# kimweiskopf/fargocpt

Measured on AMD Instinct MI355X. Metric: cell-updates/s on Nr x Nphi polar grid, higher is better.
Workload: dtype f64

## Files before the change

### fargocpt_amd/binding.py

```python
from __future__ import annotations

import ctypes as C
from typing import Optional

import numpy as np

ABI_VERSION = 5
OVERLAP = 7
GEOM_PAD = 15
MAX_BODIES = 8
NBODY_STATE = 9

SPACING_ARITHMETIC, SPACING_LOGARITHMIC, SPACING_EXPONENTIAL = 0, 1, 2
EOS_ISOTHERMAL, EOS_IDEAL = 0, 1
ARTVISC_NONE, ARTVISC_TW, ARTVISC_SN = 0, 1, 2
OPACITY_LIN, OPACITY_BELL, OPACITY_CONST, OPACITY_SIMPLE = 0, 1, 2, 3
BETAREF_ZERO, BETAREF_REFERENCE, BETAREF_MODEL, BETAREF_FLOOR = 0, 1, 2, 3
LIMITER_VANLEER, LIMITER_MC = 0, 1
INTEGRATOR_EULER, INTEGRATOR_LEAPFROG = 0, 1
(BC_ZEROGRADIENT, BC_REFERENCE, BC_REFLECTING, BC_OUTFLOW, BC_KEPLERIAN, BC_ZEROSHEAR,
 BC_NONE) = range(7)
DAMP_NONE, DAMP_REFERENCE, DAMP_ZERO, DAMP_MEAN = range(4)
IC_PROFILE, IC_SPREADING_RING, IC_SHOCKTUBE = range(3)
(F_SIGMA, F_VRAD, F_VAZI, F_ENERGY, F_PRESSURE, F_SOUNDSPEED, F_SCALE_HEIGHT, F_VISCOSITY,
 F_TEMPERATURE, F_POTENTIAL, F_SIGMA0, F_VRAD0, F_VAZI0, F_ENERGY0, F_QPLUS, F_QMINUS,
 F_VISC_CFAC_PHI, F_VISC_CFAC_R, F_MASSFLOW, F_ACCEL_RADIAL, F_ACCEL_AZIMUTHAL) = range(21)
VECTOR_FIELDS = (F_VRAD, F_VRAD0, F_MASSFLOW, F_ACCEL_RADIAL, F_ACCEL_AZIMUTHAL)
COMM_ID_BYTES = 128

ERRORS = {-1: "FCPT_EINVAL", -2: "FCPT_ENOMEM", -3: "FCPT_EHIP", -4: "FCPT_ESPLIT", -5: "FCPT_ENODEV", -6: "FCPT_ESHEAR",
          -7: "FCPT_ECOMM"}

_i32, _u32, _u64, _f64 = C.c_int32, C.c_uint32, C.c_uint64, C.c_double


class Desc(C.Structure):
    _fields_ = [
        ("struct_size", _u32), ("abi_version", _u32),
        ("nr_global", _i32), ("nphi", _i32), ("rank", _i32), ("nranks", _i32),
        ("radial_spacing", _i32), ("_pad0", _i32),
        ("rmin", _f64), ("rmax", _f64), ("exponential_cell_size_factor", _f64),
        ("eos", _i32), ("_pad1", _i32),
        ("adiabatic_index", _f64), ("mu", _f64), ("aspect_ratio", _f64), ("flaring_index", _f64),
        ("minimum_temperature", _f64), ("maximum_temperature", _f64),
        ("sigma0", _f64), ("sigma_slope", _f64), ("sigma_floor", _f64),
        ("viscous_alpha", _f64), ("constant_viscosity", _f64), ("radial_viscosity_factor", _f64),
        ("stabilize_viscosity", _i32), ("artificial_viscosity", _i32),
        ("artificial_viscosity_factor", _f64),
        ("artificial_viscosity_dissipation", _i32), ("heating_viscous", _i32),
        ("heating_viscous_factor", _f64),
        ("fast_transport", _i32), ("flux_limiter", _i32),
        ("integrator", _i32), ("_pad2", _i32),
        ("cfl", _f64), ("cfl_max_var", _f64), ("first_dt", _f64),
        ("heating_cooling_cfl_limit", _f64), ("monitor_timestep", _f64),
# ... 461 lines not shown
```

### fargocpt_amd/csrc/fcpt_context.hip

```cpp
#include "fcpt_ctx.h"

using namespace fcpt;

namespace fcpt {

void drop_graph(fcpt_ctx *c)
{
    if (c->graph_exec)
        (void)hipGraphExecDestroy(c->graph_exec);
    if (c->graph)
        (void)hipGraphDestroy(c->graph);
    c->graph_exec = nullptr;
    c->graph = nullptr;
    c->graph_cycle = 0;
}

void join_side(fcpt_ctx *c)
{
    if (c->join_pending) {
        (void)hipStreamWaitEvent(c->stream, c->e_join, 0);
        c->join_pending = false;
    }
}

int read_clock(fcpt_ctx *c, DevClock *out)
{
    join_side(c);
    HIPCHK(hipMemcpyAsync(c->h_clk, c->P.clk, sizeof(DevClock), hipMemcpyDeviceToHost, c->stream));
    HIPCHK(hipStreamSynchronize(c->stream));
    *out = *c->h_clk;
    if (out->shear_error) {
        set_error("a step exceeded the FARGO shear limit (|Nshift[i]-Nshift[i-1]| > 1) with the option "
                  "transport_fallback = 0, i.e. without the two-kernel transport queued behind the fused one; "
                  "the state is invalid");
        return FCPT_ESHEAR;
    }
    return FCPT_OK;
}

}

namespace {

int *option_slot(Options &o, const char *name)
{
#define X(n)                     \
    if (!std::strcmp(name, #n)) \
        return &o.n;
    FCPT_OPTION_NAMES
#undef X
    return nullptr;
}

void options_from_environment(Options &o)
{
    o.transport_fused = o.transport_rows = o.source_rows = o.theta_rows = -1;
    o.transport_graded = 1;
    o.source_graded = -1;
// ... 406 lines not shown
                    R.ra1sq_k = ra1 * ra1;
                    R.ra0sq_k = ra0 * ra0;
                    R.inv_rmsum_k = 1.0 / (g.Rmed[k] + g.Rmed[k - 1]);
                    R.rmed_k = g.Rmed[k];
                    R.rmed_km1 = g.Rmed[k - 1];
                    R.idr_k = at(g.InvDiffRmed, k);
                }
            }
        }
        if (!rc) rc = dev_upload_raw(c, &P.src_tab, rows);
    }

    const size_t ns = (size_t)nr * nphi, nv = (size_t)(nr + 1) * nphi;
#define AL(field, n) \
    if (!rc)         \
        rc = dev_alloc(c, &P.field, (n));
    AL(sigma, ns) AL(vrad, nv) AL(vazi, ns) AL(energy, ns) AL(vrad_b, nv) AL(vazi_b, ns) AL(energy_b, ns)
    AL(pressure, ns) AL(soundspeed, ns) AL(scale_height, ns) AL(viscosity, ns) AL(temperature, ns)
    AL(potential, ns)
    AL(sigma0, ns) AL(vrad0, nv) AL(vazi0, ns) AL(energy0, ns)
    AL(qr, ns) AL(qphi, ns) AL(divv, ns) AL(trr, ns) AL(tpp, ns) AL(trp, nv) AL(qplus, ns) AL(qminus, ns)
    AL(rmpA, ns) AL(rmmA, ns) AL(lpA, ns) AL(lmA, ns) AL(sigA, ns) AL(eA, ns)
    AL(rmpB, ns) AL(rmmB, ns) AL(lpB, ns) AL(lmB, ns) AL(sigB, ns) AL(eB, ns)
    AL(vmean, (size_t)nr + 1) AL(vconst, (size_t)nr) AL(nshift, (size_t)nr) AL(clk, 1) AL(shift_jump, 8)
    AL(cfl_part, (size_t)(nr + 256) * (size_t)((nphi + 255) / 256 + 1))
    P.ring_pstride = nphi / 32 + 4;
    AL(ring_part, (size_t)nr * P.ring_pstride)
    P.stabilize = d->stabilize_viscosity;
    if (P.stabilize) {
        AL(cfac_phi, ns) AL(cfac_r, ns)
    }
    if (d->write_massflow) {
        AL(massflow, nv)
    }
    P.accel_force = d->body_force_from_potential ? 0 : 1;
    if (P.accel_force) {
        AL(accel_r, nv) AL(accel_az, nv)
    }
    if (!rc && d->eos == FCPT_EOS_IDEAL)
        rc = dev_alloc(c, &P.qdiff, ns);
#undef AL
    if (!rc && hipHostMalloc((void **)&c->h_clk, sizeof(DevClock)) != hipSuccess) {
        set_error("hipHostMalloc failed");
        rc = FCPT_ENOMEM;
    }
    if (rc) {
        fcpt_destroy(c);
// ... 215 lines not shown
    *slot = value;
    apply_options(c, false);
    HIPCHK(hipGetLastError());
    return FCPT_OK;
}

int fcpt_get_option(const fcpt_ctx *c, const char *name, int32_t *value)
{
    if (!c || !name || !value)
        return FCPT_EINVAL;
    if (!std::strcmp(name, "graph_replays")) {
        *value = (int32_t)(c->graph_replays > 0x7fffffffll ? 0x7fffffffll : c->graph_replays);
        return FCPT_OK;
    }
    if (!std::strcmp(name, "transport_fell_back")) {
        fcpt_ctx *m = const_cast<fcpt_ctx *>(c);
        int stamps[4] = {0, 0, 0, 0};
        join_side(m);
        HIPCHK(hipMemcpyAsync(stamps, c->P.shift_jump, sizeof(stamps), hipMemcpyDeviceToHost, c->stream));
        HIPCHK(hipStreamSynchronize(c->stream));
        *value = (stamps[2] != 0 && stamps[0] == stamps[2]) ? 1 : 0;
        return FCPT_OK;
    }
    if (!std::strcmp(name, "coop_active")) {
        *value = 0;
        return FCPT_OK;
    }
    if (!std::strcmp(name, "graph_cycle")) {
        *value = c->graph_exec ? c->graph_cycle : 0;
        return FCPT_OK;
    }
    const int *slot = option_slot(const_cast<Options &>(c->P.opt), name);
    if (!slot) {
        set_error("fcpt_get_option: unknown option '%s'", name);
        return FCPT_EINVAL;
    }
    *value = *slot;
    return FCPT_OK;
}

int fcpt_set_transport_chunks(fcpt_ctx *c, const int32_t *lengths, int32_t n)
{
    if (!c || n < 0 || (n > 0 && !lengths))
        return FCPT_EINVAL;
    if (c->stepped) {
        set_error("fcpt_set_transport_chunks between fcpt_step and fcpt_post");
// ... 120 lines not shown
        *dt_max = k.dt_max;
    if (reset) {
        k.dt_min = 1.0e300;
        k.dt_max = 0.0;
        *c->h_clk = k;
        HIPCHK(hipMemcpyAsync(c->P.clk, c->h_clk, sizeof(DevClock), hipMemcpyHostToDevice, c->stream));
        HIPCHK(hipStreamSynchronize(c->stream));
    }
    return FCPT_OK;
}

int fcpt_set_clock(fcpt_ctx *c, const fcpt_clock *in)
{
    if (!c || !in)
        return FCPT_EINVAL;
    DevClock k;
    if (int rc = read_clock(c, &k))
        return rc;
    k.time = in->time;
    k.last_dt = in->last_dt;
    k.n_hydro_iter = in->n_hydro_iter;
    k.n_monitor = in->n_monitor;
    k.n_snapshot = in->n_snapshot;
    HIPCHK(hipMemsetAsync(c->P.shift_jump, 0, 8 * sizeof(int), c->stream));
    *c->h_clk = k;
    HIPCHK(hipMemcpyAsync(c->P.clk, c->h_clk, sizeof(DevClock), hipMemcpyHostToDevice, c->stream));
    HIPCHK(hipStreamSynchronize(c->stream));
    return FCPT_OK;
}

static size_t grid_count(const fcpt_ctx *c, int32_t f)
{
    const bool vec = f == FCPT_F_VRAD || f == FCPT_F_VRAD0 || f == FCPT_F_MASSFLOW || f == FCPT_F_ACCEL_RADIAL ||
                     f == FCPT_F_ACCEL_AZIMUTHAL;
    return (size_t)(c->s.nr + (vec ? 1 : 0)) * c->d.nphi;
}

int fcpt_upload(fcpt_ctx *c, int32_t f, const double *host)
{
    if (!c || !host || f < 0 || f >= FCPT_F_COUNT || !c->grid[f]) {
        set_error("bad argument to fcpt_upload");
        return FCPT_EINVAL;
    }
    join_side(c);
    HIPCHK(hipMemcpyAsync(c->grid[f], host, grid_count(c, f) * sizeof(double), hipMemcpyHostToDevice, c->stream));
    HIPCHK(hipStreamSynchronize(c->stream));
    if (f == FCPT_F_SIGMA || f == FCPT_F_VRAD || f == FCPT_F_VAZI || f == FCPT_F_ENERGY) {
// ... 329 lines not shown
```

### fargocpt_amd/csrc/fcpt_ctx.h

```cpp
#ifndef FCPT_CTX_H
#define FCPT_CTX_H

#include <hip/hip_runtime.h>

#include <cmath>
#include <cstdio>
#include <cstdlib>
#include <cstring>
#include <new>
#include <string>
#include <vector>

#include "fcpt_comm.h"
#include "fcpt_kernels.h"

using namespace fcpt;

#define HIPCHK(call)                                                                        \
    do {                                                                                    \
        hipError_t e_ = (call);                                                             \
        if (e_ != hipSuccess) {                                                             \
            set_error("%s failed: %s (%s:%d)", #call, hipGetErrorString(e_), __FILE__, __LINE__); \
            return FCPT_EHIP;                                                               \
        }                                                                                   \
// ... 6 lines not shown
    std::vector<double> radii;
    Dev P;
    hipStream_t stream = nullptr;
    std::vector<void *> allocs;
    double *d_cs_ring = nullptr;
    double *grid[FCPT_F_COUNT] = {};
    DampRange damp[4][2];
    bool potential_valid = false;
    DevClock *h_clk = nullptr;
    Profiler prof;
    bool profiling = false;
    bool fused_source = true;
    int src_parts = 0;
    bool kick_energy_b = false;
    bool kick_bc_folded = false;
    bool ghosts_unknown = true;
    bool policy_dt_dev = false;
    double policy_dt_host = -1.0;
    bool march_source = true;
    bool stepped = false;
    bool bc_deferred = false;
    bool skip_q_store = false;
    bool want_gated_deferred = false, gated_pending = false;
    GatedTheta gated;
    bool fold_pending = false;
    bool cfl_interior = false;
    bool damp_any = false;
    bool qdiff_valid = false;
    std::vector<int> ring_ref_damped;
    int *sm_sched_dev = nullptr;
    size_t sm_sched_cap = 0;
    std::vector<int> sm_sched_host;
    int *tf_sched_dev = nullptr;
    size_t tf_sched_cap = 0;
    std::vector<int> tf_lengths;
    std::vector<int> tf_sched_host;
    bool damp_foldable = false;
    hipStream_t side = nullptr;
    hipEvent_t e_fork = nullptr, e_join = nullptr;
    bool join_pending = false;
    bool pressure_valid = false;
    double *dob_part = nullptr, *dob_host = nullptr;
    hipEvent_t e_dob = nullptr;
    int dob_pending = 0;
    bool has_mid = false;
    double mx[FCPT_MAX_BODIES], my[FCPT_MAX_BODIES], mm[FCPT_MAX_BODIES], mrsm[FCPT_MAX_BODIES];
// ... 75 lines not shown
```

### fargocpt_amd/csrc/fcpt_internal.h

```cpp
#ifndef FCPT_INTERNAL_H
#define FCPT_INTERNAL_H

#include "../../include/fargocpt_hip.h"

#include <cstddef>
#include <cstdint>
#include <vector>

#ifndef M_PI
#define M_PI 3.14159265358979323846
#endif

namespace fcpt {

void set_error(const char *fmt, ...);

struct HostGeometry {
    std::vector<double> Rmed, Rinf, Rsup, Surf, InvRmed, InvRinf, InvSurf, InvDiffRmed, InvDiffRsup,
        InvDiffRsupRb;
    double dphi = 0, invdphi = 0;
    double cf_growth = 0, cf_inv_log_growth = 0, cf_opt_const = 0;
};

int build_radii(const fcpt_desc &d, double *radii);
int split_domain(const fcpt_desc &d, fcpt_split &out);
void build_geometry(const fcpt_desc &d, const fcpt_split &s, const double *radii, HostGeometry &g);
int rmed_id(const fcpt_desc &d, const fcpt_split &s, const HostGeometry &g, double r);
int rinf_id(const fcpt_desc &d, const fcpt_split &s, const HostGeometry &g, double r);

struct DevClock {
    double time;
    double last_dt;
    double dt;
    double cfl_dt;
    unsigned long long cfl_bits;
    unsigned long long n_hydro_iter;
    unsigned int n_monitor;
    unsigned int n_snapshot;
    unsigned int shear_error;
    unsigned int last_dt_pending;
    double dt_min, dt_max;
};
#ifdef __HIPCC__
__device__ __forceinline__ void clock_advance(DevClock *clk, double dt)
{
    clk->time += dt;
    clk->n_hydro_iter += 1;
    if (clk->last_dt_pending) {
        clk->last_dt = dt;
        clk->last_dt_pending = 0;
    }
    clk->dt_min = dt < clk->dt_min ? dt : clk->dt_min;
    clk->dt_max = dt > clk->dt_max ? dt : clk->dt_max;
}
#endif

struct DampRange {
    int lo, hi;
    int type;
    double rlim, redge, tau;
};

struct CArr {
    const double *p;
// ... 166 lines not shown
```

### fargocpt_amd/csrc/fcpt_kernels.h

```cpp
#ifndef FCPT_KERNELS_H
#define FCPT_KERNELS_H

#include <vector>
#include <hip/hip_runtime.h>

#include "fcpt_internal.h"
#include "fcpt_schedule.h"

namespace fcpt {

enum KernelId {
    KID_POTENTIAL, KID_SOURCE_VR, KID_SOURCE_VA, KID_COMPRESSION, KID_TW_Q, KID_TW_VA, KID_TW_VR,
    KID_SN_Q, KID_SN_E, KID_SN_VR, KID_SN_VA, KID_TRANGE, KID_ADI_CS_H, KID_ISO_CS_H,
    KID_VISCOSITY, KID_PRESSURE, KID_TEMPERATURE, KID_STRESS_DIAG, KID_STRESS_RPHI, KID_VISC_VA,
    KID_VISC_VR, KID_QPLUS, KID_SUBSTEP3, KID_BOUNDARY, KID_DAMPING, KID_TRANSPORT_RADIAL,
    KID_RING_MEAN, KID_THETA1, KID_THETA2, KID_VELOCITIES, KID_CFL_INIT, KID_CFL_CELLS, KID_CLOCK,
    KID_SRC_FUSED, KID_AV_FUSED, KID_VISC_FUSED, KID_SOURCE_MARCH, KID_THETA_MARCH,
    KID_TRANSPORT_FUSED, KID_MASSFLOW, KID_CFL_RINGS, KID_THETA_GATED_BOUNDARY, KID_EXCHANGE_COPY,
    KID_DISK_ON_BODY, KID_VISC_FACTORS, KID_SOURCE_MARCH_ADI, KID_SOURCE_MARCH_ADI_WIDE,
    KID_ACCEL_ON_GAS, KID_SOURCE_MARCH_ADI_ACC, KID_TRANSPORT_RADIAL_MEANS, KID_CFL_RINGS_BC,
    KID_DISK_ON_BODIES, KID_COUNT
};
static_assert(KID_COUNT <= 64, "fcpt_profile_start selects kernels with a 64-bit mask");
extern const char *const kKernelNames[KID_COUNT];
// ... 41 lines not shown
TransportResult launch_transport(const Dev &P, const Dev &W, hipStream_t st, int part = TRANSPORT_ALL, GatedTheta *defer_gated = nullptr);
int device_cus();
void launch_shift_means(const Dev &P, hipStream_t st);
void launch_massflow(const Dev &P, hipStream_t st);
void launch_substep3_cooling_only(const Dev &P, hipStream_t st);
void launch_disk_on_body(const Dev &P, double x, double y, double r_object, double smoothing_fixed, double r_sm, double *out,
                         hipStream_t st);
struct DiskBodies {
    double x[FCPT_MAX_BODIES], y[FCPT_MAX_BODIES], r_object[FCPT_MAX_BODIES], smoothing_fixed[FCPT_MAX_BODIES], r_sm[FCPT_MAX_BODIES];
};
size_t disk_on_bodies_blocks(const Dev &P);
void launch_disk_on_bodies(const Dev &P, int n, const DiskBodies &B, double *part, double *out, hipStream_t st);
void launch_source_fused(const Dev &P, hipStream_t st);
int launch_source_march(const Dev &P, hipStream_t st, bool fold_bc, bool *bc_folded, bool fold_cfl = false);
void launch_cfl_final(const Dev &P, int apply_policy, hipStream_t st);
bool cfl_by_rings(const Dev &P);
void launch_viscous_fused(const Dev &P, hipStream_t st);
void launch_derived(const Dev &P, hipStream_t st);
void launch_pressure(const Dev &P, hipStream_t st);
void launch_temperature(const Dev &P, hipStream_t st);
void launch_cfl(const Dev &P, int apply_policy, hipStream_t st, bool interior_done = false);
bool launch_cfl_interior(const Dev &P, hipStream_t st);
bool cfl_bc_mergeable(const Dev &P);
void launch_cfl_bc(const Dev &P, int apply_policy, hipStream_t st);
void launch_clock_set_dt(DevClock *clk, double dt, hipStream_t st);
void launch_clock_scale_dt(DevClock *clk, int mode, double dt, double factor, hipStream_t st);
void launch_clock_export_cfl(DevClock *clk, double *out, hipStream_t st);
void launch_clock_policy_ptr(DevClock *clk, double cfl_max_var, const double *cfl_global, hipStream_t st);
void launch_clock_advance(DevClock *clk, hipStream_t st);
void launch_clock_policy(DevClock *clk, double cfl_max_var, int use_device_cfl, double cfl_global,
                         hipStream_t st);

}
#endif
```

### fargocpt_amd/csrc/fcpt_step.hip

```cpp
#include "fcpt_ctx.h"

using namespace fcpt;

namespace fcpt {

void apply_boundary_view(fcpt_ctx *c, const Dev &P, bool final, bool damping_done)
{
    if (final && c->d.damping && !damping_done) {
        for (int o = 0; o < 2; ++o)
            launch_damping(P, P.vrad, P.vrad0, P.Rinf.p, c->damp[0][o], 0, c->stream);
        for (int o = 0; o < 2; ++o)
            launch_damping(P, P.vazi, P.vazi0, P.Rmed.p, c->damp[1][o], 0, c->stream);
        for (int o = 0; o < 2; ++o)
            launch_damping(P, P.sigma, P.sigma0, P.Rmed.p, c->damp[2][o], 1, c->stream);
        if (P.adiabatic)
            for (int o = 0; o < 2; ++o)
                launch_damping(P, P.energy, P.energy0, P.Rmed.p, c->damp[3][o], 0, c->stream);
    }
    launch_boundary(P, c->stream);
}
void apply_boundary(fcpt_ctx *c, bool final) { apply_boundary_view(c, c->P, final); }

void ensure_pressure(fcpt_ctx *c)
{
// ... 164 lines not shown
        c->pressure_valid = false;
        if (P.adiabatic && !P.lazy_derived)
            ensure_pressure(c);
        c->P.kick_time_shift = 1;
        const bool home = enqueue_kick(c);
        c->P.kick_time_shift = 0;
        if (home) {
            const size_t ns = (size_t)P.nr * P.nphi * sizeof(double), nv = (size_t)(P.nr + 1) * P.nphi * sizeof(double);
            (void)hipMemcpyAsync(P.vrad, P.vrad_b, nv, hipMemcpyDeviceToDevice, st);
            (void)hipMemcpyAsync(P.vazi, P.vazi_b, ns, hipMemcpyDeviceToDevice, st);
            if (c->kick_energy_b)
                (void)hipMemcpyAsync(P.energy, P.energy_b, ns, hipMemcpyDeviceToDevice, st);
            c->kick_energy_b = false;
        }
        launch_clock_scale_dt(P.clk, 2, 0.0, 1.0, st);
    }
    c->stepped = true;
}

void flush_deferred_boundary(fcpt_ctx *c)
{
    if (c->bc_deferred) {
        c->bc_deferred = false;
        launch_boundary(c->P, c->stream);
    }
}

void enqueue_post(fcpt_ctx *c, bool may_defer_boundary)
{
    join_side(c);
    const bool damping_done = c->P.damp_in_step != 0 && c->stepped;
    const bool defer = may_defer_boundary && (damping_done || !c->damp_any) && !(c->P.adiabatic && !c->P.lazy_derived) && cfl_bc_mergeable(c->P);
    if (c->gated_pending) {
        c->gated_pending = false;
        if (!defer && (damping_done || !c->d.damping)) {
            launch_gated_theta(c->gated, &c->P, c->stream);
            c->stepped = false;
            if (c->P.adiabatic && !c->P.lazy_derived) {
                launch_derived(c->P, c->stream);
                c->pressure_valid = true;
            } else {
                c->pressure_valid = false;
            }
            return;
        }
        launch_gated_theta(c->gated, nullptr, c->stream);
    }
    if (defer)
        c->bc_deferred = true;
    else
        apply_boundary_view(c, c->P, true, damping_done);
    c->stepped = false;
    if (c->P.adiabatic && !c->P.lazy_derived) {
        launch_derived(c->P, c->stream);
        c->pressure_valid = true;
    } else {
        c->pressure_valid = false;
    }
}

void enqueue_cfl(fcpt_ctx *c, int apply_policy)
{
    join_side(c);
    c->P.qdiff_on = c->qdiff_valid ? 1 : 0;
    if (c->bc_deferred && !c->cfl_interior && cfl_bc_mergeable(c->P)) {
        c->bc_deferred = false;
        launch_cfl_bc(c->P, apply_policy, c->stream);
    } else {
        flush_deferred_boundary(c);
        launch_cfl(c->P, apply_policy, c->stream, c->cfl_interior);
    }
    c->cfl_interior = false;
}

}

extern "C" {

int fcpt_cfl_begin(fcpt_ctx *c)
{
    if (!c)
        return FCPT_EINVAL;
    join_side(c);
    c->cfl_interior = false;
    const bool state_final = c->stepped && (!c->damp_any || c->P.damp_in_step != 0);
    if (!state_final)
        return FCPT_OK;
    if (c->P.opt.cfl_split == 0)
        return FCPT_OK;
    ProfScope prof_scope(c);
// ... 141 lines not shown
    return FCPT_OK;
}

int fcpt_apply_boundary(fcpt_ctx *c, double dt, int32_t final)
{
    if (!c)
        return FCPT_EINVAL;
    join_side(c);
    ProfScope prof_scope(c);
    launch_clock_set_dt(c->P.clk, dt, c->stream);
    apply_boundary(c, final != 0);
    HIPCHK(hipGetLastError());
    return FCPT_OK;
}

}
namespace {
unsigned launch_flags(const fcpt_ctx *c)
{
    return (c->potential_valid ? 1u : 0u) | (c->pressure_valid ? 2u : 0u) | (c->stepped ? 4u : 0u) |
           (c->cfl_interior ? 8u : 0u) | (c->kick_energy_b ? 16u : 0u) | (c->fused_source ? 32u : 0u) |
           (c->march_source ? 64u : 0u) | (c->has_mid ? 128u : 0u) | (c->join_pending ? 256u : 0u) |
           (c->ghosts_unknown ? 1024u : 0u) | (c->qdiff_valid ? 2048u : 0u) |
           (c->bc_deferred ? 4096u : 0u) | ((unsigned)c->src_parts << 13);
}
bool graph_wanted(const fcpt_ctx *c)
{
    if (c->profiling || c->graph_failed || c->comm)
        return false;
    if (c->P.opt.graph_steps >= 0)
        return c->P.opt.graph_steps != 0;
    return (long long)c->P.nr * c->P.nphi <= 131072;
}
void enqueue_device_step(fcpt_ctx *c)
{
    const bool frog = c->d.integrator == FCPT_INTEGRATOR_LEAPFROG;
    const int want = c->P.opt.cfl_fold_in_source;
    const bool fold = (want < 0 ? (long long)c->P.nr * c->P.nphi < (1ll << 22) : want != 0) && !frog && c->fused_source &&
                      c->march_source && source_march_applies(c->P) && cfl_by_rings(c->P);
    enqueue_cfl(c, fold ? 2 : 1);
    c->fold_pending = fold;
    {
        const bool pure_bc = (c->P.damp_in_step != 0 || !c->d.damping) && !(c->P.adiabatic && !c->P.lazy_derived);
        const bool rides_in_cfl = c->P.opt.bc_in_cfl != 0 && (c->P.damp_in_step != 0 || !c->damp_any) &&
                                  !(c->P.adiabatic && !c->P.lazy_derived) && cfl_bc_mergeable(c->P);
        c->want_gated_deferred = c->P.opt.gate_in_boundary != 0 && !frog && pure_bc && !rides_in_cfl;
    }
    enqueue_step(c, true, 0.0, c->d.cfl <= 0.8);
    enqueue_post(c, c->P.opt.bc_in_cfl != 0);
}
bool capture_graph(fcpt_ctx *c, int cycle)
{
    if (!c->capture_stream && hipStreamCreateWithFlags(&c->capture_stream, hipStreamNonBlocking) != hipSuccess)
        return false;
    const Dev P0 = c->P;
    const unsigned f0 = launch_flags(c);
    hipStream_t user = c->stream;
    c->stream = c->capture_stream;
    bool ok = hipStreamBeginCapture(c->capture_stream, hipStreamCaptureModeThreadLocal) == hipSuccess;
    if (ok) {
        for (int n = 0; n < cycle; ++n)
            enqueue_device_step(c);
        hipGraph_t g = nullptr;
        ok = hipStreamEndCapture(c->capture_stream, &g) == hipSuccess && g != nullptr;
        c->graph = g;
    }
    c->stream = user;
    (void)hipGetLastError();
    const bool periodic = std::memcmp(&P0, &c->P, sizeof(Dev)) == 0 && f0 == launch_flags(c);
    if (ok && periodic)
        ok = hipGraphInstantiate(&c->graph_exec, c->graph, nullptr, nullptr, 0) == hipSuccess;
    if (!ok || !periodic) {
        c->P = P0;
        c->grid[FCPT_F_SIGMA] = c->P.sigma;
        c->grid[FCPT_F_VRAD] = c->P.vrad;
        c->grid[FCPT_F_VAZI] = c->P.vazi;
        c->grid[FCPT_F_ENERGY] = c->P.energy;
        c->potential_valid = f0 & 1u;
        c->pressure_valid = f0 & 2u;
        c->stepped = f0 & 4u;
        c->cfl_interior = f0 & 8u;
        c->kick_energy_b = f0 & 16u;
        c->ghosts_unknown = f0 & 1024u;
        c->qdiff_valid = f0 & 2048u;
        c->bc_deferred = f0 & 4096u;
        c->src_parts = (int)(f0 >> 13);
        drop_graph(c);
        return false;
    }
    c->graph_cycle = cycle;
    c->graph_P = c->P;
    c->graph_flags = f0;
    return true;
}
}
extern "C" {

int fcpt_run_steps(fcpt_ctx *c, int64_t nsteps, int32_t snap, int64_t *done)
{
    if (!c)
        return FCPT_EINVAL;
    ProfScope prof_scope(c);
    int64_t n = 0;
    const bool slabs = c->comm && (c->peer_inner >= 0 || c->peer_outer >= 0);
    if (slabs && !snap) {
        for (; n < nsteps; ++n) {
            if (int rc = enqueue_cfl_allreduce(c))
                return rc;
// ... 104 lines not shown
```

### fargocpt_amd/csrc/kernels/cfl.h

```cpp

#include "../fcpt_schedule.h"
template <bool ROWU> __global__ void k_cfl_cells(const Dev P, double *part, int rows)
{
    const int j = blockIdx.x * blockDim.x + threadIdx.x;
    const int r0_ = P.first_active + (blockIdx.y * blockDim.y + threadIdx.y) * rows;
    const int r0 = ROWU ? __builtin_amdgcn_readfirstlane(r0_) : r0_;
    double s = 0.0;
    if (j < P.nphi && r0 < P.active_size) {
        const int jn = JNEXT;
        const int r1 = r0 + rows < P.active_size ? r0 + rows : P.active_size;
        const double lf = P.leapfrog ? 0.6 : 1.0;
        const double C2 = P.art_visc_factor * P.art_visc_factor;
        const double gg1 = P.gamma * (P.gamma - 1.0), inv_sqrt_gamma = 1.0 / sqrt(P.gamma);
        const double inv_limit = 1.0 / P.heating_cooling_cfl_limit;
        double vr0 = P.vrad[IDX(r0, j)];
        for (int i = r0; i < r1; ++i) {
            const double vr1 = P.vrad[IDX(i + 1, j)];
            const double inv_dxr = P.InvDiffRsup[i];
            const double inv_dxa = P.InvRmed[i] * P.invdphi;
            const double inv_cell = dmax(inv_dxr, inv_dxa);
            const double va = P.vazi[IDX(i, j)];
            const double van = P.vazi[IDX(i, jn)];
            const double vres = P.fast_transport ? va - P.vmean_c[i] : va;
            double cs, nu;
// ... 171 lines not shown
            }
        }
    }
    for (int off = 32; off > 0; off >>= 1)
        s = dmax(s, __shfl_down(s, off, 64));
    if ((t & 63) == 0)
        s_m[t >> 6] = s;
    __syncthreads();
    if (t == 0) {
        double m = dmax(dmax(s_m[0], s_m[1]), dmax(s_m[2], s_m[3]));
#pragma unroll
        for (int q = 4; q < NW; ++q)
            m = dmax(m, s_m[q]);
        part[i] = m;
    }
}
#define CFL_RINGS_ATTR __launch_bounds__(NT)
template <bool ADI, int MAXP, int NT = 256> __global__ void CFL_RINGS_ATTR k_cfl_rings(const Dev P, double *part, int r1, int n1, int r2)
{
    const int b = xcd_block(blockIdx.x, gridDim.x);
    const int i = b < n1 ? r1 + b : r2 + (b - n1);
    cfl_ring_block<ADI, MAXP, NT, (NT >= 512)>(P, part, i);
}
template <bool ADI, int MAXP, int NT = 256> __global__ void CFL_RINGS_ATTR k_cfl_rings_bc(const Dev P, double *part, int nbc)
{
    const int b = blockIdx.x, t = threadIdx.x;
    int *flag = P.shift_jump;
    const int seq = SHIFT_SEQ(P.clk);
    if (b < nbc) {
        const int j = b * NT + t;
        if (j < P.nphi)
            boundary_column(P, j, 3);
        __syncthreads();
        if (t == 0) {
            __threadfence();
            if (__hip_atomic_fetch_add(flag + 1, 1, __ATOMIC_ACQ_REL, __HIP_MEMORY_SCOPE_AGENT) == nbc - 1) {
                __hip_atomic_store(flag + 1, 0, __ATOMIC_RELAXED, __HIP_MEMORY_SCOPE_AGENT);
                __hip_atomic_store(flag + 3, seq, __ATOMIC_RELEASE, __HIP_MEMORY_SCOPE_AGENT);
            }
        }
        return;
    }
    const int nr = P.nr, nfree = nr - 4, q = b - nbc;
    int i;
    if (q < nfree) {
        i = 2 + xcd_block(q, nfree);
    } else {
        const int d = q - nfree;
        i = d == 0 ? 0 : (d == 1 ? 1 : (d == 2 ? nr - 2 : nr - 1));
        while (__hip_atomic_load(flag + 3, __ATOMIC_ACQUIRE, __HIP_MEMORY_SCOPE_AGENT) != seq)
            __builtin_amdgcn_s_sleep(2);
    }
    cfl_ring_block<ADI, MAXP, NT, (NT >= 512)>(P, part, i);
}
__device__ __forceinline__ double cfl_fold_value(const Dev &P, const double *part, int nparts)
{
    double smax = 0.0;
    for (int n = threadIdx.x; n < nparts; n += blockDim.x)
        smax = dmax(smax, part[n]);
    double dmx = 0.0;
    for (int n = threadIdx.x; n < P.active_size; n += blockDim.x) {
        if (n == 0 || n >= P.first_active) {
            const double denom = fabs(P.vmean[n] * P.InvRmed[n] - P.vmean[n + 1] * P.InvRmed[n + 1]) + 1.0e-100;
            dmx = dmax(dmx, denom);
        }
    }
    for (int off = 32; off > 0; off >>= 1) {
        smax = dmax(smax, __shfl_down(smax, off, 64));
        dmx = dmax(dmx, __shfl_down(dmx, off, 64));
    }
    __shared__ double s_s[16], s_d[16];
    const int wave = threadIdx.x >> 6, lane = threadIdx.x & 63;
    if (lane == 0) {
        s_s[wave] = smax;
        s_d[wave] = dmx;
    }
// ... 83 lines not shown
```

### fargocpt_amd/csrc/kernels/device_util.h

```cpp

#define IDX(i, j) ((i) * P.nphi + (j))

struct Launch2D {
    dim3 grid, block;
};
static inline Launch2D launch2d(int nrows, int nphi)
{
    int bx = 1;
    while (bx < nphi && bx < 256)
        bx <<= 1;
    const int by = 256 / bx;
    Launch2D l;
    l.block = dim3(bx, by, 1);
    l.grid = dim3((nphi + bx - 1) / bx, (nrows + by - 1) / by, 1);
    return l;
}
#define CELL(row0, nrows)                                            \
    const int j = blockIdx.x * blockDim.x + threadIdx.x;             \
    const int i_ = (row0) + blockIdx.y * blockDim.y + threadIdx.y;   \
    if (j >= P.nphi || i_ >= (row0) + (nrows))                       \
        return;                                                      \
    const int i = ROWU ? __builtin_amdgcn_readfirstlane(i_) : i_;
#define JNEXT (j == P.nphi - 1 ? 0 : j + 1)
#define JPREV (j == 0 ? P.nphi - 1 : j - 1)
// ... 103 lines not shown
    int lo = __double2loint(x), hi = __double2hiint(x);
    const int slo = __builtin_amdgcn_update_dpp(0, lo, CTRL, ROW_MASK, 0xf, true);
    const int shi = __builtin_amdgcn_update_dpp(0, hi, CTRL, ROW_MASK, 0xf, true);
    return x + __hiloint2double(shi, slo);
}
__device__ __forceinline__ double wave_sum(double x)
{
    x = dpp_add<0x111, 0xf>(x);
    x = dpp_add<0x112, 0xf>(x);
    x = dpp_add<0x114, 0xf>(x);
    x = dpp_add<0x118, 0xf>(x);
    x = dpp_add<0x142, 0xa>(x);
    x = dpp_add<0x143, 0xc>(x);
    return x;
}

#define SHIFT_SEQ(clk_) ((int)(((clk_)->n_hydro_iter + 1ull) & 0x7fffffffull))
__device__ __forceinline__ bool shift_jump_raised(const int *flag)
{
    const int __attribute__((address_space(4))) *f = (const int __attribute__((address_space(4))) *)flag;
    return f[0] == f[2];
}

__device__ __forceinline__ double ld_off(const double *base, unsigned off) { return *(const double *)((const char *)base + off); }
__device__ __forceinline__ void st_off(double *base, unsigned off, double v) { *(double *)((char *)base + off) = v; }
__device__ __forceinline__ D2 ld2_off(const double *base, unsigned off) { return LD2((const double *)((const char *)base + off)); }
__device__ __forceinline__ void st2_off(double *base, unsigned off, D2 v) { ST2((double *)((char *)base + off), v); }


#define MARCH_WAVES 4

__device__ __forceinline__ double cfl_fold_in_step(const Dev &P);
```

### fargocpt_amd/csrc/kernels/launch.h

```cpp

const char *const kKernelNames[KID_COUNT] = {
    "k_potential", "k_source_vr", "k_source_va", "k_compression_heating", "k_tw_q", "k_tw_va", "k_tw_vr",
    "k_sn_q", "k_sn_e", "k_sn_vr", "k_sn_va", "k_temperature_range", "k_adi_derived", "k_iso_cs_h",
    "k_viscosity", "k_pressure", "k_temperature", "k_stress_diag", "k_stress_rphi", "k_visc_va",
    "k_visc_vr", "k_qplus_qminus", "k_substep3", "k_boundary", "k_damping", "k_transport_radial",
    "k_ring_mean", "k_transport_theta<1>", "k_transport_theta<2>", "k_velocities", "k_cfl_final",
    "k_cfl_cells", "k_clock", "k_src_fused", "k_av_fused", "k_visc_fused", "k_source_march",
    "k_transport_theta_march", "k_transport_fused", "k_massflow", "k_cfl_rings", "k_theta_march_gated_boundary",
    "k_exchange_copy", "k_disk_on_body", "k_visc_factors", "k_source_march_adi", "k_source_march_adi_wide",
    "k_accel_on_gas", "k_source_march_adi_acc",
    "k_transport_radial_means", "k_cfl_rings_bc", "k_disk_on_bodies"};

thread_local Profiler *g_prof = nullptr;

void Profiler::begin(int id, hipStream_t st)
{
    if (!((mask >> id) & 1ull) || used + 2 > (int)events.size())
        return;
    if (stride > 1 && (seen++ % stride) != 0)
        return;
    (void)hipEventRecord(events[used], st);
    open_id = id;
}
void Profiler::end(int id, hipStream_t st)
// ... 464 lines not shown
            f(ADI, int_c<CFL_MAXP / 2>{}, int_c<512>{});
        else if (wide)
            f(ADI, int_c<2 * CFL_MAXP>{}, int_c<256>{});
        else
            f(ADI, int_c<CFL_MAXP>{}, int_c<256>{});
    });
}
static void launch_cfl_rings(const Dev &P, int r1, int n1, int r2, int n2, hipStream_t st)
{
    if (n1 + n2 <= 0)
        return;
    with_cfl_ring_shape(P, [&](auto ADI, auto MAXP, auto NT) {
        KLAUNCH(KID_CFL_RINGS, (k_cfl_rings<TARG(ADI), TARG(MAXP), TARG(NT)>), dim3(n1 + n2), dim3(TARG(NT)), P, P.cfl_part, r1, n1, r2);
    });
}
bool cfl_bc_mergeable(const Dev &P)
{
    return cfl_by_rings(P) && P.nr >= 8 && ((long long)P.nr * P.nphi >= (1ll << 22) || P.opt.bc_in_cfl == 2);
}
static void launch_cfl_fold(const Dev &P, int nparts, int apply_policy, hipStream_t st)
{
    KLAUNCH(KID_CFL_INIT, k_cfl_final, dim3(1), dim3(1024), P, (const double *)P.cfl_part, nparts, apply_policy);
}
void launch_cfl_bc(const Dev &P, int apply_policy, hipStream_t st)
{
    with_cfl_ring_shape(P, [&](auto ADI, auto MAXP, auto NT) {
        const int nbc = (P.nphi + TARG(NT) - 1) / TARG(NT);
        KLAUNCH(KID_CFL_RINGS_BC, (k_cfl_rings_bc<TARG(ADI), TARG(MAXP), TARG(NT)>), dim3(nbc + P.nr), dim3(TARG(NT)), P, P.cfl_part, nbc);
    });
    if (apply_policy != 2)
        launch_cfl_final(P, apply_policy, st);
}
void launch_cfl_final(const Dev &P, int apply_policy, hipStream_t st) { launch_cfl_fold(P, P.nr, apply_policy, st); }
bool launch_cfl_interior(const Dev &P, hipStream_t st)
{
    if (!cfl_by_rings(P) || P.nr <= CFL_EDGE_LO + CFL_EDGE_HI)
        return false;
    launch_cfl_rings(P, CFL_EDGE_LO, P.nr - CFL_EDGE_LO - CFL_EDGE_HI, 0, 0, st);
    return true;
}
void launch_cfl(const Dev &P, int apply_policy, hipStream_t st, bool interior_done)
{
    if (cfl_by_rings(P)) {
        if (interior_done)
            launch_cfl_rings(P, 0, CFL_EDGE_LO, P.nr - CFL_EDGE_HI, CFL_EDGE_HI, st);
        else
            launch_cfl_rings(P, 0, P.nr, 0, 0, st);
        if (apply_policy != 2)
            launch_cfl_final(P, apply_policy, st);
        return;
    }
// ... 38 lines not shown
```

### include/fargocpt_hip.h

```cpp
#ifndef FARGOCPT_HIP_H
#define FARGOCPT_HIP_H

#include <stdint.h>

#ifdef __cplusplus
extern "C" {
#endif

#define FCPT_ABI_VERSION 5

#define FCPT_OK 0
#define FCPT_EINVAL -1
#define FCPT_ENOMEM -2
#define FCPT_EHIP -3
#define FCPT_ESPLIT -4
#define FCPT_ENODEV -5
#define FCPT_ESHEAR -6
#define FCPT_ECOMM -7

#define FCPT_OVERLAP 7
#define FCPT_GHOSTCELLS_B 1
#define FCPT_GEOM_PAD 15
#define FCPT_MAX_BODIES 8

enum { FCPT_SPACING_ARITHMETIC = 0, FCPT_SPACING_LOGARITHMIC = 1, FCPT_SPACING_EXPONENTIAL = 2 };
enum { FCPT_EOS_ISOTHERMAL = 0, FCPT_EOS_IDEAL = 1 };
enum { FCPT_ARTVISC_NONE = 0, FCPT_ARTVISC_TW = 1, FCPT_ARTVISC_SN = 2 };
enum { FCPT_LIMITER_VANLEER = 0, FCPT_LIMITER_MC = 1 };
enum { FCPT_OPACITY_LIN = 0, FCPT_OPACITY_BELL = 1, FCPT_OPACITY_CONST = 2, FCPT_OPACITY_SIMPLE = 3 };
enum { FCPT_BETAREF_ZERO = 0, FCPT_BETAREF_REFERENCE = 1, FCPT_BETAREF_MODEL = 2, FCPT_BETAREF_FLOOR = 3 };
enum { FCPT_INTEGRATOR_EULER = 0, FCPT_INTEGRATOR_LEAPFROG = 1 };
enum {
    FCPT_BC_ZEROGRADIENT = 0,
    FCPT_BC_REFERENCE = 1,
    FCPT_BC_REFLECTING = 2,
    FCPT_BC_OUTFLOW = 3,
    FCPT_BC_KEPLERIAN = 4,
    FCPT_BC_ZEROSHEAR = 5,
    FCPT_BC_NONE = 6
};
enum { FCPT_DAMP_NONE = 0, FCPT_DAMP_REFERENCE = 1, FCPT_DAMP_ZERO = 2, FCPT_DAMP_MEAN = 3 };
// ... 291 lines not shown
```

Before: 26.62 billion.

## Fold gated theta-march fallback into the merged CFL/boundary kernel launch

When the boundary is deferred into the CFL ring kernel, the gated FARGO theta-march fallback is now also deferred and run by extra leading workgroups of that same kernel. The remaining CFL/boundary workgroups wait on a stamp those workgroups publish. The aim is to remove a separate kernel launch and its serialization per step. The cost is an intra-launch spin-wait that relies on workgroup co-residency. To limit that risk it adds a bounded wait with a sync_error flag and a new ESYNC error code, and caps waves per EU on the new variant.

```diff
diff --git a/fargocpt_amd/binding.py b/fargocpt_amd/binding.py
--- a/fargocpt_amd/binding.py
+++ b/fargocpt_amd/binding.py
@@ -29,7 +29,7 @@
 COMM_ID_BYTES = 128
 
 ERRORS = {-1: "FCPT_EINVAL", -2: "FCPT_ENOMEM", -3: "FCPT_EHIP", -4: "FCPT_ESPLIT", -5: "FCPT_ENODEV", -6: "FCPT_ESHEAR",
-          -7: "FCPT_ECOMM"}
+          -7: "FCPT_ECOMM", -8: "FCPT_ESYNC"}
 
 _i32, _u32, _u64, _f64 = C.c_int32, C.c_uint32, C.c_uint64, C.c_double
 
diff --git a/fargocpt_amd/csrc/fcpt_context.hip b/fargocpt_amd/csrc/fcpt_context.hip
--- a/fargocpt_amd/csrc/fcpt_context.hip
+++ b/fargocpt_amd/csrc/fcpt_context.hip
@@ -34,6 +34,10 @@
                   "transport_fallback = 0, i.e. without the two-kernel transport queued behind the fused one; "
                   "the state is invalid");
         return FCPT_ESHEAR;
+    }
+    if (out->sync_error) {
+        set_error("a workgroup's bounded wait for a stamp of its own launch ran out (k_cfl_rings_bc); the state is invalid");
+        return FCPT_ESYNC;
     }
     return FCPT_OK;
 }
@@ -486,7 +490,7 @@
     AL(qr, ns) AL(qphi, ns) AL(divv, ns) AL(trr, ns) AL(tpp, ns) AL(trp, nv) AL(qplus, ns) AL(qminus, ns)
     AL(rmpA, ns) AL(rmmA, ns) AL(lpA, ns) AL(lmA, ns) AL(sigA, ns) AL(eA, ns)
     AL(rmpB, ns) AL(rmmB, ns) AL(lpB, ns) AL(lmB, ns) AL(sigB, ns) AL(eB, ns)
-    AL(vmean, (size_t)nr + 1) AL(vconst, (size_t)nr) AL(nshift, (size_t)nr) AL(clk, 1) AL(shift_jump, 8)
+    AL(vmean, (size_t)nr + 1) AL(vconst, (size_t)nr) AL(nshift, (size_t)nr) AL(clk, 1) AL(shift_jump, 16)
     AL(cfl_part, (size_t)(nr + 256) * (size_t)((nphi + 255) / 256 + 1))
     P.ring_pstride = nphi / 32 + 4;
     AL(ring_part, (size_t)nr * P.ring_pstride)
@@ -748,6 +752,15 @@
         *value = (stamps[2] != 0 && stamps[0] == stamps[2]) ? 1 : 0;
         return FCPT_OK;
     }
+    if (!std::strcmp(name, "gated_in_cfl_seq")) {
+        fcpt_ctx *m = const_cast<fcpt_ctx *>(c);
+        int stamps[8] = {0, 0, 0, 0, 0, 0, 0, 0};
+        join_side(m);
+        HIPCHK(hipMemcpyAsync(stamps, c->P.shift_jump, sizeof(stamps), hipMemcpyDeviceToHost, c->stream));
+        HIPCHK(hipStreamSynchronize(c->stream));
+        *value = stamps[6];
+        return FCPT_OK;
+    }
     if (!std::strcmp(name, "coop_active")) {
         *value = 0;
         return FCPT_OK;
@@ -914,7 +927,7 @@
     k.n_hydro_iter = in->n_hydro_iter;
     k.n_monitor = in->n_monitor;
     k.n_snapshot = in->n_snapshot;
-    HIPCHK(hipMemsetAsync(c->P.shift_jump, 0, 8 * sizeof(int), c->stream));
+    HIPCHK(hipMemsetAsync(c->P.shift_jump, 0, 16 * sizeof(int), c->stream));
     *c->h_clk = k;
     HIPCHK(hipMemcpyAsync(c->P.clk, c->h_clk, sizeof(DevClock), hipMemcpyHostToDevice, c->stream));
     HIPCHK(hipStreamSynchronize(c->stream));
diff --git a/fargocpt_amd/csrc/fcpt_ctx.h b/fargocpt_amd/csrc/fcpt_ctx.h
--- a/fargocpt_amd/csrc/fcpt_ctx.h
+++ b/fargocpt_amd/csrc/fcpt_ctx.h
@@ -52,6 +52,7 @@
     bool bc_deferred = false;
     bool skip_q_store = false;
     bool want_gated_deferred = false, gated_pending = false;
+    bool gated_deferred = false;
     GatedTheta gated;
     bool fold_pending = false;
     bool cfl_interior = false;
diff --git a/fargocpt_amd/csrc/fcpt_internal.h b/fargocpt_amd/csrc/fcpt_internal.h
--- a/fargocpt_amd/csrc/fcpt_internal.h
+++ b/fargocpt_amd/csrc/fcpt_internal.h
@@ -40,6 +40,8 @@
     unsigned int shear_error;
     unsigned int last_dt_pending;
     double dt_min, dt_max;
+    unsigned int sync_error;
+    unsigned int pad_;
 };
 #ifdef __HIPCC__
 __device__ __forceinline__ void clock_advance(DevClock *clk, double dt)
diff --git a/fargocpt_amd/csrc/fcpt_kernels.h b/fargocpt_amd/csrc/fcpt_kernels.h
--- a/fargocpt_amd/csrc/fcpt_kernels.h
+++ b/fargocpt_amd/csrc/fcpt_kernels.h
@@ -87,7 +87,7 @@
 void launch_cfl(const Dev &P, int apply_policy, hipStream_t st, bool interior_done = false);
 bool launch_cfl_interior(const Dev &P, hipStream_t st);
 bool cfl_bc_mergeable(const Dev &P);
-void launch_cfl_bc(const Dev &P, int apply_policy, hipStream_t st);
+void launch_cfl_bc(const Dev &P, int apply_policy, hipStream_t st, const GatedTheta *gated = nullptr);
 void launch_clock_set_dt(DevClock *clk, double dt, hipStream_t st);
 void launch_clock_scale_dt(DevClock *clk, int mode, double dt, double factor, hipStream_t st);
 void launch_clock_export_cfl(DevClock *clk, double *out, hipStream_t st);
diff --git a/fargocpt_amd/csrc/fcpt_step.hip b/fargocpt_amd/csrc/fcpt_step.hip
--- a/fargocpt_amd/csrc/fcpt_step.hip
+++ b/fargocpt_amd/csrc/fcpt_step.hip
@@ -210,7 +210,12 @@
 {
     if (c->bc_deferred) {
         c->bc_deferred = false;
-        launch_boundary(c->P, c->stream);
+        if (c->gated_deferred) {
+            c->gated_deferred = false;
+            launch_gated_theta(c->gated, &c->P, c->stream);
+        } else {
+            launch_boundary(c->P, c->stream);
+        }
     }
 }
 
@@ -221,7 +226,9 @@
     const bool defer = may_defer_boundary && (damping_done || !c->damp_any) && !(c->P.adiabatic && !c->P.lazy_derived) && cfl_bc_mergeable(c->P);
     if (c->gated_pending) {
         c->gated_pending = false;
-        if (!defer && (damping_done || !c->d.damping)) {
+        if (defer) {
+            c->gated_deferred = true;
+        } else if (damping_done || !c->d.damping) {
             launch_gated_theta(c->gated, &c->P, c->stream);
             c->stepped = false;
             if (c->P.adiabatic && !c->P.lazy_derived) {
@@ -231,8 +238,9 @@
                 c->pressure_valid = false;
             }
             return;
-        }
-        launch_gated_theta(c->gated, nullptr, c->stream);
+        } else {
+            launch_gated_theta(c->gated, nullptr, c->stream);
+        }
     }
     if (defer)
         c->bc_deferred = true;
@@ -253,7 +261,8 @@
     c->P.qdiff_on = c->qdiff_valid ? 1 : 0;
     if (c->bc_deferred && !c->cfl_interior && cfl_bc_mergeable(c->P)) {
         c->bc_deferred = false;
-        launch_cfl_bc(c->P, apply_policy, c->stream);
+        launch_cfl_bc(c->P, apply_policy, c->stream, c->gated_deferred ? &c->gated : nullptr);
+        c->gated_deferred = false;
     } else {
         flush_deferred_boundary(c);
         launch_cfl(c->P, apply_policy, c->stream, c->cfl_interior);
@@ -441,7 +450,7 @@
            (c->cfl_interior ? 8u : 0u) | (c->kick_energy_b ? 16u : 0u) | (c->fused_source ? 32u : 0u) |
            (c->march_source ? 64u : 0u) | (c->has_mid ? 128u : 0u) | (c->join_pending ? 256u : 0u) |
            (c->ghosts_unknown ? 1024u : 0u) | (c->qdiff_valid ? 2048u : 0u) |
-           (c->bc_deferred ? 4096u : 0u) | ((unsigned)c->src_parts << 13);
+           (c->bc_deferred ? 4096u : 0u) | (c->gated_deferred ? 512u : 0u) | ((unsigned)c->src_parts << 13);
 }
 bool graph_wanted(const fcpt_ctx *c)
 {
@@ -461,9 +470,7 @@
     c->fold_pending = fold;
     {
         const bool pure_bc = (c->P.damp_in_step != 0 || !c->d.damping) && !(c->P.adiabatic && !c->P.lazy_derived);
-        const bool rides_in_cfl = c->P.opt.bc_in_cfl != 0 && (c->P.damp_in_step != 0 || !c->damp_any) &&
-                                  !(c->P.adiabatic && !c->P.lazy_derived) && cfl_bc_mergeable(c->P);
-        c->want_gated_deferred = c->P.opt.gate_in_boundary != 0 && !frog && pure_bc && !rides_in_cfl;
+        c->want_gated_deferred = c->P.opt.gate_in_boundary != 0 && !frog && pure_bc;
     }
     enqueue_step(c, true, 0.0, c->d.cfl <= 0.8);
     enqueue_post(c, c->P.opt.bc_in_cfl != 0);
@@ -473,6 +480,7 @@
     if (!c->capture_stream && hipStreamCreateWithFlags(&c->capture_stream, hipStreamNonBlocking) != hipSuccess)
         return false;
     const Dev P0 = c->P;
+    const GatedTheta G0 = c->gated;
     const unsigned f0 = launch_flags(c);
     hipStream_t user = c->stream;
     c->stream = c->capture_stream;
@@ -503,6 +511,8 @@
         c->ghosts_unknown = f0 & 1024u;
         c->qdiff_valid = f0 & 2048u;
         c->bc_deferred = f0 & 4096u;
+        c->gated_deferred = f0 & 512u;
+        c->gated = G0;
         c->src_parts = (int)(f0 >> 13);
         drop_graph(c);
         return false;
diff --git a/fargocpt_amd/csrc/kernels/cfl.h b/fargocpt_amd/csrc/kernels/cfl.h
--- a/fargocpt_amd/csrc/kernels/cfl.h
+++ b/fargocpt_amd/csrc/kernels/cfl.h
@@ -217,10 +217,43 @@
     const int i = b < n1 ? r1 + b : r2 + (b - n1);
     cfl_ring_block<ADI, MAXP, NT, (NT >= 512)>(P, part, i);
 }
-template <bool ADI, int MAXP, int NT = 256> __global__ void CFL_RINGS_ATTR k_cfl_rings_bc(const Dev P, double *part, int nbc)
-{
-    const int b = blockIdx.x, t = threadIdx.x;
+struct NoGatedMarch {
+    static constexpr bool on = false;
+};
+template <bool DAMP> struct GatedMarch {
+    static constexpr bool on = true, damp = DAMP;
+    Dev Wm;
+    const double *va_pre, *vr_pre;
+    ThetaSet in;
+    int tiles, rows, nvb, ntheta;
+};
+template <bool ADI, int MAXP, int NT, class G> __device__ __forceinline__ void cfl_rings_bc_body(const Dev &P, double *part, int nbc, const G &g)
+{
+    int b = blockIdx.x;
+    const int t = threadIdx.x;
     int *flag = P.shift_jump;
+    if constexpr (G::on) {
+        const bool raised = shift_jump_raised(flag);
+        if (b < g.ntheta) {
+            if (!raised)
+                return;
+            for (int vb = b; vb < g.nvb; vb += g.ntheta)
+                transport_theta_march_block<2, ADI, G::damp, false>(g.Wm, g.va_pre, g.vr_pre, g.in, g.tiles, g.rows, 0, vb, g.nvb);
+            __syncthreads();
+            if (t == 0) {
+                __threadfence();
+                if (__hip_atomic_fetch_add(flag + 4, 1, __ATOMIC_ACQ_REL, __HIP_MEMORY_SCOPE_AGENT) == g.ntheta - 1) {
+                    __hip_atomic_store(flag + 4, 0, __ATOMIC_RELAXED, __HIP_MEMORY_SCOPE_AGENT);
+                    flag[6] = flag[2];
+                    __hip_atomic_store(flag + 5, flag[2], __ATOMIC_RELEASE, __HIP_MEMORY_SCOPE_AGENT);
+                }
+            }
+            return;
+        }
+        b -= g.ntheta;
+        if (raised && !wait_for_stamp(flag + 5, flag[2], P.clk))
+            return;
+    }
     const int seq = SHIFT_SEQ(P.clk);
     if (b < nbc) {
         const int j = b * NT + t;
@@ -243,10 +276,24 @@
     } else {
         const int d = q - nfree;
         i = d == 0 ? 0 : (d == 1 ? 1 : (d == 2 ? nr - 2 : nr - 1));
-        while (__hip_atomic_load(flag + 3, __ATOMIC_ACQUIRE, __HIP_MEMORY_SCOPE_AGENT) != seq)
-            __builtin_amdgcn_s_sleep(2);
+        if (!wait_for_stamp(flag + 3, seq, P.clk))
+            return;
     }
     cfl_ring_block<ADI, MAXP, NT, (NT >= 512)>(P, part, i);
+}
+template <bool ADI, int MAXP, int NT = 256> __global__ void CFL_RINGS_ATTR k_cfl_rings_bc(const Dev P, double *part, int nbc)
+{
+    cfl_rings_bc_body<ADI, MAXP, NT>(P, part, nbc, NoGatedMarch{});
+}
+template <bool ADI, int MAXP, int NT> constexpr int cfl_bc_waves()
+{
+    return ADI ? (NT >= 512 || MAXP > CFL_MAXP ? 3 : 5) : (NT >= 512 ? 5 : (MAXP > CFL_MAXP ? 4 : 6));
+}
+template <bool ADI, int MAXP, int NT, bool DAMP>
+__global__ void CFL_RINGS_ATTR __attribute__((amdgpu_waves_per_eu(cfl_bc_waves<ADI, MAXP, NT>(), cfl_bc_waves<ADI, MAXP, NT>())))
+k_cfl_rings_bc(const Dev P, double *part, int nbc, const GatedMarch<DAMP> g)
+{
+    cfl_rings_bc_body<ADI, MAXP, NT>(P, part, nbc, g);
 }
 __device__ __forceinline__ double cfl_fold_value(const Dev &P, const double *part, int nparts)
 {
diff --git a/fargocpt_amd/csrc/kernels/device_util.h b/fargocpt_amd/csrc/kernels/device_util.h
--- a/fargocpt_amd/csrc/kernels/device_util.h
+++ b/fargocpt_amd/csrc/kernels/device_util.h
@@ -149,6 +149,18 @@
     return f[0] == f[2];
 }
 
+#define STAMP_WAIT_POLLS (1 << 24)
+__device__ __forceinline__ bool wait_for_stamp(const int *word, int seq, DevClock *clk)
+{
+    for (int n = 0; n < STAMP_WAIT_POLLS; ++n) {
+        if (__hip_atomic_load(word, __ATOMIC_ACQUIRE, __HIP_MEMORY_SCOPE_AGENT) == seq)
+            return true;
+        __builtin_amdgcn_s_sleep(2);
+    }
+    clk->sync_error = 1;
+    return false;
+}
+
 __device__ __forceinline__ double ld_off(const double *base, unsigned off) { return *(const double *)((const char *)base + off); }
 __device__ __forceinline__ void st_off(double *base, unsigned off, double v) { *(double *)((char *)base + off) = v; }
 __device__ __forceinline__ D2 ld2_off(const double *base, unsigned off) { return LD2((const double *)((const char *)base + off)); }
diff --git a/fargocpt_amd/csrc/kernels/launch.h b/fargocpt_amd/csrc/kernels/launch.h
--- a/fargocpt_amd/csrc/kernels/launch.h
+++ b/fargocpt_amd/csrc/kernels/launch.h
@@ -510,11 +510,27 @@
 {
     KLAUNCH(KID_CFL_INIT, k_cfl_final, dim3(1), dim3(1024), P, (const double *)P.cfl_part, nparts, apply_policy);
 }
-void launch_cfl_bc(const Dev &P, int apply_policy, hipStream_t st)
+void launch_cfl_bc(const Dev &P, int apply_policy, hipStream_t st, const GatedTheta *gated)
 {
     with_cfl_ring_shape(P, [&](auto ADI, auto MAXP, auto NT) {
         const int nbc = (P.nphi + TARG(NT) - 1) / TARG(NT);
-        KLAUNCH(KID_CFL_RINGS_BC, (k_cfl_rings_bc<TARG(ADI), TARG(MAXP), TARG(NT)>), dim3(nbc + P.nr), dim3(TARG(NT)), P, P.cfl_part, nbc);
+        if (!gated) {
+            KLAUNCH(KID_CFL_RINGS_BC, (k_cfl_rings_bc<TARG(ADI), TARG(MAXP), TARG(NT)>), dim3(nbc + P.nr), dim3(TARG(NT)), P, P.cfl_part, nbc);
+            return;
+        }
+        const Dev &T = gated->P, &Wm = gated->Wm;
+        const ThetaGeometry tg = theta_geometry(T, 2, 0);
+        constexpr int NW = TARG(NT) / 64;
+        const int nvb = (((T.nr + tg.rows - 1) / tg.rows) * tg.tiles + NW - 1) / NW;
+        const int ntheta = nvb > FALLBACK_BLOCKS ? FALLBACK_BLOCKS : nvb;
+        with_bool(Wm.damp_in_step, [&](auto DD) {
+            GatedMarch<TARG(DD)> g;
+            g.Wm = Wm, g.va_pre = T.vazi, g.vr_pre = T.vrad;
+            g.in = ThetaSet{T.rmpB, T.rmmB, T.lpB, T.lmB, T.sigB, T.eB};
+            g.tiles = tg.tiles, g.rows = tg.rows, g.nvb = nvb, g.ntheta = ntheta;
+            KLAUNCH(KID_CFL_RINGS_BC, (k_cfl_rings_bc<TARG(ADI), TARG(MAXP), TARG(NT), TARG(DD)>), dim3(ntheta + nbc + P.nr), dim3(TARG(NT)), P,
+                    P.cfl_part, nbc, g);
+        });
     });
     if (apply_policy != 2)
         launch_cfl_final(P, apply_policy, st);
diff --git a/include/fargocpt_hip.h b/include/fargocpt_hip.h
--- a/include/fargocpt_hip.h
+++ b/include/fargocpt_hip.h
@@ -17,6 +17,7 @@
 #define FCPT_ENODEV -5
 #define FCPT_ESHEAR -6
 #define FCPT_ECOMM -7
+#define FCPT_ESYNC -8
 
 #define FCPT_OVERLAP 7
 #define FCPT_GHOSTCELLS_B 1
```

New measurement: 26.38 billion. About the same (-0.9%).
